# oma219/spumoni

Measured on AMD Instinct MI355X. Metric: reads/s PML classification, 200 bp reads vs 10-hap human index, higher is better.
Workload: dtype u64

## Files before the change

### spumoni_amd/csrc/spx_internal.h

```cpp
#pragma once
#include <hip/hip_runtime.h>

#include <memory>
#include <functional>
#include <mutex>
#include <string>
#include <vector>

#include "../../include/spumoni_gpu.h"
#include "spx_layout.h"

namespace spx {

void set_error(const char* fmt, ...);
int hip_fail(hipError_t e, const char* what, const char* file, int line);
int select_device(int device);

#define SPX_HIP(call)                                                        \
    do {                                                                     \
        hipError_t e_ = (call);                                              \
        if (e_ != hipSuccess) return spx::hip_fail(e_, #call, __FILE__, __LINE__); \
    } while (0)

struct QuietOnError {
// ... 59 lines not shown
    uint32_t* read_fail;
    const uint64_t* chunk_start;
    WalkState* reentry;
    uint64_t* vtop;
    uint32_t* pending;
    uint32_t round;
    uint32_t last_round;
};
constexpr uint32_t CHUNK_TOP = 0x80000000u, CHUNK_BOTTOM = 0x40000000u, CHUNK_ACTIVE = 0x20000000u;
constexpr uint32_t CHUNK_LEN_MASK = 0x1fffffffu;
constexpr int CHUNK_EXTRA_ROUNDS = 3;

struct BatchArgs {
    const uint8_t* seqs;
    const uint64_t* offs;
    uint64_t nreads;
    uint64_t total_chars;
    uint32_t* out_lengths;
    uint64_t* out_pointers;
    uint32_t* out_docs;
    spx_class* out_class;
    uint64_t bin_width;
    uint64_t bin_magic;
    uint64_t max_value_thr;
    WalkCounters* counters;
    uint32_t lanes_per_wave;
    uint32_t narrow;
    ChunkArgs ch;
    const uint32_t* only_flagged;
    const uint64_t* in_starts;
    uint64_t* len_mask;
    unsigned long long* claim;
    uint64_t len_mask_pairs;
};

}

struct spc_params;

namespace spx {
struct ArrayOwner {
    int device = 0;
    void* p[10] = {};
    ~ArrayOwner() {
        (void)hipSetDevice(device);
        for (void* a : p)
            if (a) (void)hipFree(a);
    }
};
}

struct spx_index {
    int device = 0;
    uint64_t n = 0, r = 0;
    bool has_samples = false, has_docs = false;
    spx::Row* rows = nullptr;
    uint32_t* q_alloc = nullptr;
    spx::JumpRow* dirrows = nullptr;
    char* fat = nullptr;
    uint32_t* fat_js = nullptr;
    spx::Aux* aux = nullptr;
    uint64_t* ss_by_run = nullptr;
    uint32_t* rundocs = nullptr;
    spx::LetterInfo* letters = nullptr;
    uint8_t* text = nullptr;
    uint64_t n_text = 0;
    static constexpr int NARR = 10;
    uint64_t arr_bytes[NARR] = {};
    std::shared_ptr<spx::ArrayOwner> owner;
    hipStream_t ctx_stream = nullptr;
    static constexpr int NDIGSCR = 15;
    hipEvent_t ev_dig = nullptr;
    hipStream_t dig_stream = nullptr;
    bool dig_used = false;
    spx::DevIndex view{};
    spx::WalkCounters* counters = nullptr;
    bool claim_used = false;
    hipEvent_t ev0 = nullptr, ev1 = nullptr, ev_done = nullptr;
    bool have_timing = false;
    hipStream_t last_stream = nullptr;
    uint64_t device_bytes = 0;
    int waves_per_cu = 0;
    int occ_blocks[8] = {};
    int num_cus = 0;
    int force_lanes_per_wave = 0;
    int force_digest_kernel = 0;
    int digest_parked = 0;
    uint8_t charhash[4] = {0, 0, 0, 0};
    char source_tag[128] = {0};
    static constexpr int PIPE_CHUNKS = 10;
    hipStream_t pipe_s[3] = {nullptr, nullptr, nullptr};
    hipEvent_t pipe_in[PIPE_CHUNKS] = {}, pipe_k[PIPE_CHUNKS] = {};
    std::mutex mu;
    std::mutex host_mu;
    struct Scratch {
        void* p = nullptr;
        size_t cap = 0;
        hipError_t grow(size_t bytes, void** out) {
            if (cap < bytes) {
                if (p) (void)hipFree(p);
                p = nullptr;
                cap = 0;
                const size_t want = bytes + bytes / 4 + 256;
                const hipError_t e = hipMalloc(&p, want);
                if (e != hipSuccess) return e;
                cap = want;
            }
            *out = p;
            return hipSuccess;
        }
        int reserve(size_t bytes, void** out) {
            SPX_HIP(grow(bytes, out));
            return SPX_OK;
        }
    };
    enum { S_SEQ, S_OFFS, S_LEN, S_PTR, S_DOC, S_CLASS, S_RAW, S_DIG_OFFS, S_GAP, S_SCAN,
           S_LINE_BYTES, S_LINE_START = S_LINE_BYTES + 3, S_TEXT = S_LINE_START + 3, S_COUNT = S_TEXT + 3 };
    static constexpr int reads_slot(int digest_kind) { return digest_kind ? S_RAW : S_SEQ; }
    Scratch scratch[S_COUNT];
    enum { C_DESC, C_ENDS, C_SEAMS, C_CKPT, C_FLAGS, C_FAIL, C_CNT, C_CUB, C_LEN_BITS, C_COUNT };
    Scratch chunk_scr[C_COUNT];
    Scratch digest_scr[NDIGSCR];
    enum { G_RAW, G_OFFS, G_DIG, G_DIG_OFFS, G_LEN, G_DOC, G_PTR, G_SET_STRIDE, G_COUNT = 2 * G_SET_STRIDE };
    Scratch stage_scr[G_COUNT];
    hipStream_t stage_s[2] = {nullptr, nullptr};
    struct Product {
        Scratch counters;
        hipEvent_t ev0 = nullptr, ev1 = nullptr;
        hipStream_t stream = nullptr;
        bool have = false, pending = false;
        uint64_t acc[6] = {};
        uint64_t error = 0;
        float ms = 0;
    };
    enum { V_MEDIUM, V_LONG, V_TILES, V_ACC, V_TABLE, V_OUT0, V_COUNT = V_OUT0 + 2 };
    Scratch vote_scr[V_COUNT];
    Product votes;
    enum { M_COUNTERS, M_BITS, M_PREFIX, M_CUB, M_MOFFS, M_OUT, M_OUT_DOCS, M_COUNT };
    Scratch mems_scr[M_COUNT];
    hipEvent_t ev_m[4] = {nullptr, nullptr, nullptr, nullptr};
    hipStream_t mems_stream = nullptr;
    bool have_mems = false, mems_pending = false, mems_ready = false, mems_ready_docs = false;
    uint64_t mems_capacity = 0, mems_ready_n = 0;
    uint64_t mems_acc[4] = {};
    float mems_ms = 0;
    Scratch place_scr[2];
    Product place;
    enum { H_OUT, H_COUNT };
    Scratch chain_scr[H_COUNT];
    Product chain;
    enum { L_CNT, L_GOFFS, L_GAPS, L_DESC, L_LIST, L_CUB, L_CHAINS, L_OUT, L_PRED, L_COUNT };
    Scratch align_scr[L_COUNT];
    Product align;
    hipEvent_t ev_align[3] = {nullptr, nullptr, nullptr};
    bool align_steps = false;
    float align_step_ms[4] = {};
    enum { TB_CNT, TB_GOFFS, TB_GAPS, TB_DESC, TB_LIST, TB_CUB, TB_PW, TB_POFFS, TB_PATH, TB_TRACE, TB_OCNT, TB_CHAINS, TB_OUT,
           TB_PRED, TB_OOFFS, TB_OPS, TB_EPW, TB_EPOFFS, TB_ERES, TB_ETRACE, TB_ENDS, TB_COUNT };
    Scratch cigar_scr[TB_COUNT];
    Product cigar;
    hipEvent_t ev_cigar[7] = {};
    bool cigar_phase[2] = {false, false};
    float cigar_step_ms[5] = {};
    uint64_t cigar_extra[4] = {};
    bool cigar_ready = false;
    uint64_t cigar_ready_n = 0, cigar_ready_reads = 0;
// ... 168 lines not shown
```

### spumoni_amd/csrc/spx_walk.hip

```cpp
#include <hipcub/hipcub.hpp>

#include <type_traits>

#include "spx_internal.h"

namespace spx {

namespace {

enum : uint32_t {
    P_READ = 0,
    P_CHARS = 1,
    P_LAND = 2,
    P_FAT = 3,
    P_QS = 4,
    P_DIR = 5,
    P_AUX = 6,
    P_SAMP = 7,
    P_FATJ = 8,
    P_DONE = 9,
    P_START = 10,
    P_CKPT = 11
};

// ... 870 lines not shown
    uint32_t k = (uint32_t)k_start;
    uint64_t off = 0;
    for (uint64_t guard = 0;; ++guard) {
        const Row row = row_at(ix, k);
        const uint32_t H = ix.compact ? crow_H(row) : row_H(row);
        if (t < n_text) text[t] = (uint8_t)H;
        uint32_t k0 = ix.compact ? crow_LFrun(row) : row_LFrun(row);
        uint64_t offp = (ix.compact ? (uint64_t)crow_LFoff(row) : row_LFoff(row)) + off;
        for (;;) {
            const Row r0 = row_at(ix, k0);
            const uint64_t len = ix.compact ? (uint64_t)crow_len(r0) : row_len(r0);
            if (offp < len || k0 >= ix.r) break;
            offp -= len;
            k0++;
        }
        if ((offp == 0 && !(ix.compact && crow_cont(row_at(ix, k0)))) || k0 >= ix.r) break;
        if (guard > ix.n) {
            atomicAdd(stuck, 1ull);
            break;
        }
        k = k0;
        off = offp;
        t -= 1;
    }
}

template <int MODE, bool DOC, bool COMPACT, bool NARROW, int CHUNK = 0>
int launch_lanes(spx_index* ix, const BatchArgs& args, hipStream_t stream, uint64_t items = 0, bool* wrote_lengths = nullptr) {
    if (CHUNK == 0) items = args.nreads;
    if (CHUNK == 0 && MODE == SPX_MODE_PML && args.out_lengths != nullptr && args.len_mask == nullptr) {
        set_error("internal: PML walk without prepare_len_mask");
        return SPX_E_ARG;
    }
    static const bool old_walk = getenv("SPX_OLD_WALK") != nullptr;
    const bool fast = COMPACT && args.only_flagged == nullptr && !old_walk && items < (1ull << 31);
    if (args.in_starts != nullptr && !(fast && CHUNK == 0)) {
        set_error("internal: parked reads (BatchArgs::in_starts) are taken by the plain k_walk_fast only");
        return SPX_E_ARG;
    }
    const int slot = (fast ? 4 : 0) + MODE * 2 + (DOC ? 1 : 0);
    if (ix->occ_blocks[slot] == 0) {
        int occ = 0;
        if (fast)
            SPX_HIP(hipOccupancyMaxActiveBlocksPerMultiprocessor(&occ, k_walk_fast<MODE, DOC, NARROW, 0>, WALK_TPB, 0));
        else
            SPX_HIP(hipOccupancyMaxActiveBlocksPerMultiprocessor(&occ, k_walk_lanes<MODE, DOC, COMPACT, NARROW, 0>, WALK_TPB, 0));
        ix->occ_blocks[slot] = occ < 1 ? 1 : occ;
    }
    if (ix->num_cus == 0) {
        hipDeviceProp_t prop;
        SPX_HIP(hipGetDeviceProperties(&prop, ix->device));
        ix->num_cus = prop.multiProcessorCount;
    }
    int occ = ix->occ_blocks[slot];
    constexpr bool SIDE = (MODE == SPX_MODE_MS) || DOC;
    const int auto_waves = ix->view.nletters > 16 ? (fast ? (SIDE ? 12 : 16) : 20) : (fast && SIDE ? 12 : 16);
    const int target_waves = ix->waves_per_cu > 0 ? ix->waves_per_cu : auto_waves;
    int want = target_waves / (WALK_TPB / 64);
    if (want < 1) want = 1;
    if (want < occ) occ = want;
    uint64_t grid = (uint64_t)occ * ix->num_cus;
    const uint64_t need = (items + WALK_TPB - 1) / WALK_TPB;
    BatchArgs a = args;
    a.lanes_per_wave = 64;
    bool small_batch = false;
    if (ix->force_lanes_per_wave > 0) {
        const uint64_t lpw = (uint64_t)(ix->force_lanes_per_wave > 64 ? 64 : ix->force_lanes_per_wave);
        a.lanes_per_wave = (uint32_t)lpw;
        const uint64_t waves_needed = (items + lpw - 1) / lpw;
        const uint64_t waves_resident = grid * (WALK_TPB / 64);
        const uint64_t waves = waves_needed < waves_resident ? waves_needed : waves_resident;
        grid = (waves + (WALK_TPB / 64) - 1) / (WALK_TPB / 64);
    } else if (need < grid) {
        small_batch = true;
        const uint64_t waves = (uint64_t)ix->num_cus * 4 * 2;
        uint64_t lpw = (items + waves - 1) / waves;
        if (lpw < 1) lpw = 1;
        if (lpw > 64) lpw = 64;
        a.lanes_per_wave = (uint32_t)lpw;
        grid = (items + lpw * 4 - 1) / (lpw * 4);
    }
    const bool dynamic = fast && CHUNK == 0 && ix->force_lanes_per_wave == 0 && !small_batch && items > grid * WALK_TPB;
    if (dynamic) {
        a.claim = &ix->counters->claim;
        if (ix->claim_used) SPX_HIP(hipMemsetAsync(a.claim, 0, sizeof(unsigned long long), stream));
        ix->claim_used = true;
    }
    if (!dynamic && ix->force_lanes_per_wave == 0 && need >= grid) {
        const uint64_t lanes_all = grid * WALK_TPB;
        const uint64_t rounds = (items + lanes_all - 1) / lanes_all;
        const uint64_t even = (items + rounds * WALK_TPB - 1) / (rounds * WALK_TPB);
        if (rounds <= 8 && even < grid && even * 8 >= grid * 7) grid = even;
    }
    if (grid == 0) grid = 1;
    if (fast) {
        if (dynamic)
            k_walk_fast<MODE, DOC, NARROW, 0, false, true><<<(unsigned)grid, WALK_TPB, 0, stream>>>(ix->view, a);
        else if (CHUNK == 2 || small_batch)
            k_walk_fast<MODE, DOC, NARROW, CHUNK, true><<<(unsigned)grid, WALK_TPB, 0, stream>>>(ix->view, a);
        else
            k_walk_fast<MODE, DOC, NARROW, CHUNK, false><<<(unsigned)grid, WALK_TPB, 0, stream>>>(ix->view, a);
        if (wrote_lengths) *wrote_lengths = MODE == SPX_MODE_PML;
    } else
        k_walk_lanes<MODE, DOC, COMPACT, NARROW, CHUNK><<<(unsigned)grid, WALK_TPB, 0, stream>>>(ix->view, a);
    SPX_HIP(hipGetLastError());
    return SPX_OK;
}


__global__ void k_chunk_count(const uint64_t* offs, uint64_t nreads, uint32_t L, int narrow, uint64_t* cnt,
                              uint32_t* read_fail, WalkCounters* counters) {
    const uint64_t q = blockIdx.x * (uint64_t)WALK_TPB + threadIdx.x;
    if (q > nreads) return;
    if (q == nreads) {
        cnt[q] = 0;
        return;
    }
    const uint64_t base = offs[q], m = offs[q + 1] - base;
    cnt[q] = m ? (base + m - 1) / L - base / L + 1 : 0;
    read_fail[q] = 0;
    if (narrow && m >= 65536) atomicAdd(&counters->error, 1ull);
}

__global__ void k_chunk_fill(const uint64_t* offs, uint64_t nreads, uint32_t L, const uint64_t* chunk_start,
                             ChunkDesc* desc, uint64_t* nchunks) {
    const uint64_t q = blockIdx.x * (uint64_t)WALK_TPB + threadIdx.x;
    if (q >= nreads) return;
    if (q == 0) *nchunks = chunk_start[nreads];
    const uint64_t base = offs[q], end = offs[q + 1];
    uint64_t c = chunk_start[q];
    for (uint64_t a = base; a < end; ++c) {
        uint64_t e = (a / L + 1) * L;
        if (e > end) e = end;
        ChunkDesc d;
        d.gend = e;
        d.len = (uint32_t)(e - a) | (e == end ? CHUNK_TOP : 0u) | (a == base ? CHUNK_BOTTOM : 0u);
        d.rd = (uint32_t)q;
        desc[c] = d;
        a = e;
    }
}

__global__ void k_chunk_scan(ChunkArgs ch, uint64_t nreads, uint32_t round, uint32_t last, WalkCounters* counters) {
    const uint64_t q = blockIdx.x * (uint64_t)WALK_TPB + threadIdx.x;
    if (q >= nreads) return;
    const uint64_t cs = ch.chunk_start[q], ce = ch.chunk_start[q + 1];
    if (ce - cs < 2) return;
    ChunkDesc* desc = const_cast<ChunkDesc*>(ch.desc);
    uint64_t j = round == 1 ? ce - 1 : ch.vtop[q];
    if (j == cs) return;
    if (round > 1) desc[j - 1].len &= ~CHUNK_ACTIVE;
    while (j > cs) {
        const uint64_t nx = j - 1;
        const SeamRec sr = ch.seams[nx];
        j = nx;
        if (nx == cs || (sr.met & 1)) continue;
        if (!last) {
            WalkState st = sr.ext;
            const ChunkDesc below = desc[nx - 1];
            const SeamRec old = ch.seams[nx - 1];
            st.flags = (uint32_t)(old.t - (below.gend - (below.len & CHUNK_LEN_MASK)));
            ch.reentry[nx - 1] = st;
            desc[nx - 1].len = below.len | CHUNK_ACTIVE;
            atomicAdd(&ch.pending[round + 1], 1u);
        }
        break;
// ... 545 lines not shown
```

### spumoni_amd/csrc/spx_walk_fast.inc

```

enum : uint32_t { Q_LAND = 0, Q_FAT = 1, Q_STEP = 2, Q_READ = 3, Q_CHARS = 4, Q_FATJ = 5, Q_QS = 6, Q_DIR = 7, Q_DONE = 8, Q_SAMP = 9, Q_START = 10, Q_WANT = 11 };
enum : uint32_t {
    F_EMB = 1,
    F_NOROW = 2,
    F_QUIRK = 4,
    F_WIDE = 16,
    F_FADD = 32,
    F_HAVEC = 64,
    F_SAMPD = 128
};
enum : uint32_t { A_STEP = 1, A_EMIT = 2, A_DECIDE = 4 };
#ifndef SPX_STEP_REPS
#define SPX_STEP_REPS 2
#endif
constexpr int STEP_REPS = SPX_STEP_REPS;
constexpr uint32_t OFF_LAST32 = 0xffffffffu;
#ifndef SPX_CHUNK_CLAIM
#define SPX_CHUNK_CLAIM 64
#endif
constexpr uint32_t CHUNK_CLAIM = SPX_CHUNK_CLAIM;
static_assert(CHUNK_CLAIM >= 64, "a claim covers at least one iteration's worst case: 64 lanes ending a read each");

__device__ __forceinline__ uint32_t dpp_swap1(uint32_t v) { return (uint32_t)__builtin_amdgcn_mov_dpp((int)v, 0xB1, 0xf, 0xf, true); }

struct alignas(16) HotLetter {
    uint32_t bmul;
    uint32_t present;
    uint64_t fat0;
};

__device__ __forceinline__ void lf_target_ct(uint32_t LFrun, uint32_t LFoff, uint32_t cums, uint32_t off, uint32_t& k0,
                                             uint32_t& offp, uint32_t& t_out) {
    lf_target_c(LFrun, LFoff, cums, off, k0, offp);
    const uint32_t t = k0 - LFrun;
    t_out = (t < 4 && off <= 126) ? t : 4u;
}

template <int MODE, bool DOC, bool NARROW, int CHUNK = 0, bool EARLY = false, bool DYN = false>
__global__ void __launch_bounds__(WALK_TPB) k_walk_fast(const DevIndex ix, const BatchArgs b) {
    constexpr bool AUX = (MODE == SPX_MODE_MS) || DOC;
    constexpr bool PML = MODE == SPX_MODE_PML;
    if (CHUNK == 2 && b.ch.round > 1 && b.ch.pending[b.ch.round] == 0) return;
    __shared__ HotLetter s_hot[256];
#ifndef SPX_PGRP
#define SPX_PGRP 16
#endif
    constexpr int PGRP = SPX_PGRP, PROW = WALK_TPB + 1;
    constexpr int PLPG = PGRP / 2, PNG = 64 / PLPG;
    __shared__ uint64_t s_ptrs[MODE == SPX_MODE_MS && CHUNK != 2 ? PGRP * PROW : 1];
    constexpr bool DSTAGE = PML && DOC && CHUNK != 2;
    constexpr int DGRP = 32, DROW = DGRP + 2;
    __shared__ uint16_t s_docs[DSTAGE ? WALK_TPB * DROW : 1];
    const LetterInfo* const s_let = ix.letters;
    __shared__ uint32_t s_win[8 * WALK_TPB];
    const char* const rows_b = reinterpret_cast<const char*>(ix.rows);
    const char* const fat_b = reinterpret_cast<const char*>(ix.fat);
    const uint32_t fs = ix.fat_stride;
    const bool lrow = !AUX && fs == 32 && ix.aux == nullptr;
    for (int t = threadIdx.x; t < 256; t += blockDim.x) {
        const LetterInfo li = ix.letters[t];
        s_hot[t] = HotLetter{li.bmul, li.qbeg != li.qend ? 1u : 0u, (uint64_t)(uintptr_t)(fat_b + li.fbase * fs)};
    }
    __syncthreads();
    const char* const dir_b = reinterpret_cast<const char*>(ix.dirrows);
    const char* const fatj_b = reinterpret_cast<const char*>(ix.fat_js);
    const char* const q_b = reinterpret_cast<const char*>(ix.Q);
    const char* const seq_b = reinterpret_cast<const char*>(b.seqs);
    const char* const off_b = reinterpret_cast<const char*>(b.offs);
    const uint32_t R = ix.r;
    const uint32_t fs_shift = fs == 32 ? 5 : 4;
    const bool want_class = PML && CHUNK == 0 && b.out_class != nullptr;
    const bool want_len = PML && CHUNK != 2 && b.out_lengths != nullptr;
    const uint32_t lpw = b.lanes_per_wave;
    const uint32_t nlanes = (uint32_t)((((uint64_t)gridDim.x * blockDim.x) >> 6) * lpw);
    const uint32_t nitems = CHUNK ? (uint32_t)*b.ch.nchunks : (uint32_t)b.nreads;
    const uint64_t ch_org = CHUNK ? b.offs[0] : 0;
    uint8_t* const ch_flags = CHUNK ? b.ch.flags - (ch_org & ~7ull) : nullptr;
    WalkState* const ch_ckpt = CHUNK ? b.ch.ckpt - (ch_org >> CKPT_SHIFT) : nullptr;
    const char* const item_b = CHUNK ? reinterpret_cast<const char*>(b.ch.desc) : off_b;
    constexpr uint32_t ITEM_BYTES = CHUNK ? sizeof(ChunkDesc) : 8;
    const uint32_t tid = threadIdx.x;
    static_assert(!DYN || (CHUNK == 0 && !EARLY), "only the plain, full launch deals its reads on demand");
    uint32_t w_n0 = 0, w_e0 = 0, w_n1 = 0, w_e1 = 0;
    bool w_pend = false;
    bool w_dry = false;
    uint32_t w_wait = DYN ? (uint32_t)((((uint64_t)blockIdx.x * blockDim.x + tid) >> 6) & 31u) + 1u : 0u;
    unsigned long long claimed = 0;

    uint32_t rd = (uint32_t)((((uint64_t)blockIdx.x * blockDim.x + tid) >> 6) * lpw) + (tid & 63);
    uint32_t ph = (rd < nitems && (tid & 63) < lpw) ? Q_READ : Q_DONE;
    const char* addr = ph == Q_READ ? item_b + (uint64_t)rd * ITEM_BYTES : item_b;
    uint32_t seen = 0;
    uint64_t fb = 0;
    uint32_t fl = 0;
    uint32_t c = 0;
    uint64_t base = 0, ibase = 0;
    uint32_t m = 0, x = 0;
    int32_t wi = -1;
    uint64_t q0 = 0, q1 = 0;
    uint32_t k = 0, off = 0;
    uint32_t length = 0;
    uint64_t mbits = 0;
    uint32_t nr = 0;
    uint32_t bin_lo = 0, bin_max = 0, above = 0, below = 0;
    uint64_t sum_max = 0;
    uint64_t sample = 0;
    uint32_t doc = 0;
    uint32_t w_jumps = 0, w_pred = 0, w_rows = 0, w_dir = 0, w_again = 0;
    uint32_t tlimit = 0xffffffffu;
    V16 cka{0, 0, 0, 0}, ckb{0, 0, 0, 0};

#define WIN_AT(w) ((s_win[((uint32_t)(w) >> 2) * WALK_TPB + tid] >> (((uint32_t)(w) & 3) * 8)) & 0xffu)
#define CUR_C c
#define COUNT(var, cond) (var += (uint32_t)__popcll(__builtin_amdgcn_ballot_w64(cond)))

    V16 ga{0, 0, 0, 0}, gb{0, 0, 0, 0};
    uint32_t side_doc = 0;
    Aux side_aux{0, 0};
    uint64_t side_in = 0;
    auto issue_gather = [&]() {
        ga = V16{0, 0, 0, 0};
        gb = V16{0, 0, 0, 0};
#ifndef SPX_PAIR_MIN
#define SPX_PAIR_MIN 24
#endif
        constexpr int pair_min = EARLY ? 65 : SPX_PAIR_MIN;
        if ((int)__popcll(__builtin_amdgcn_ballot_w64(ph != Q_DONE && (fl & F_WIDE))) < pair_min) {
            if (ph != Q_DONE) {
                ga = *reinterpret_cast<const V16*>(addr);
                if (fl & F_WIDE) gb = *reinterpret_cast<const V16*>(addr + 16);
            }
        } else
        {
            typedef uint32_t u32x4 __attribute__((ext_vector_type(4), aligned(4)));
            typedef const __attribute__((address_space(1))) u32x4* GV16;
            const bool odd = tid & 1;
            const bool live = ph != Q_DONE;
            const uint32_t w_own = (live && (fl & F_WIDE)) ? 16u : 0u;
            const uint64_t au = (uint64_t)(uintptr_t)(live ? addr : rows_b);
            const uint64_t pu = u64of(dpp_swap1((uint32_t)au), dpp_swap1((uint32_t)(au >> 32))) + 16;
            const uint32_t w_for = dpp_swap1(w_own);
            const uint64_t a1 = odd ? pu : au, a2 = odd ? au : pu;
            const bool do1 = odd ? w_for != 0 : live, do2 = odd ? live : w_for != 0;
            uint32_t r1x = 0, r1y = 0, r1z = 0, r1w = 0, r2x = 0, r2y = 0, r2z = 0, r2w = 0;
            if (do1) {
                const u32x4 t = *(GV16)(uintptr_t)a1;
                r1x = t.x, r1y = t.y, r1z = t.z, r1w = t.w;
            }
            if (do2) {
                const u32x4 t = *(GV16)(uintptr_t)a2;
                r2x = t.x, r2y = t.y, r2z = t.z, r2w = t.w;
            }
            ga = V16{odd ? r2x : r1x, odd ? r2y : r1y, odd ? r2z : r1z, odd ? r2w : r1w};
            const uint32_t zx = dpp_swap1(odd ? r1x : r2x), zy = dpp_swap1(odd ? r1y : r2y), zz = dpp_swap1(odd ? r1z : r2z),
                           zw = dpp_swap1(odd ? r1w : r2w);
            gb = V16{w_own ? zx : 0u, w_own ? zy : 0u, w_own ? zz : 0u, w_own ? zw : 0u};
        }
        side_doc = 0;
        side_aux = Aux{0, 0};
        side_in = 0;
        claimed = 0;
        if (CHUNK == 0 && b.in_starts != nullptr && ph == Q_READ) side_in = b.in_starts[rd];
        if (DOC && ph == Q_SAMP) side_doc = ix.rundocs[k];
        if (AUX && ph == Q_DIR) side_aux = ix.aux[length];
        if (DYN && w_pend && (tid & 63) == 0) claimed = atomicAdd(b.claim, (unsigned long long)CHUNK_CLAIM);
    };
    if (EARLY) issue_gather();
    while (__builtin_amdgcn_ballot_w64(ph != Q_DONE) != 0) {
        if (!EARLY) issue_gather();
        uint32_t act = 0, hd = 0;
        uint32_t rflag = 0;
        bool pred_ev = false;
        uint32_t d_trun = 0, d_toff = 0, d_srun = 0, d_soff = 0, d_bits = 0;
        Aux d_aux{0, 0};
        bool d_lrow = false;
        uint64_t fbits = 0;
        uint32_t fxi = 0;
        bool flush = false;
        bool pflush = false, pheld = false, pheld_end = false;
        uint32_t pfxi = 0;
        uint64_t phold = 0;
        COUNT(w_rows, ph == Q_LAND);
        COUNT(w_dir, ph == Q_FAT || (ph >= Q_FATJ && ph <= Q_DIR));

        if (ph == Q_LAND) {
            const uint32_t len = ga.x & 0xffffu;
            const uint32_t o = off == OFF_LAST32 ? len - 1 : off;
            if (o >= len) {
                off = o - len;
                k++;
                addr += sizeof(Row32);
            } else {
                off = o;
                q0 = u64of(ga.x, ga.y);
                q1 = u64of(ga.z, ga.w);
                fl = (fl & ~F_NOROW) | F_EMB;
                act = A_STEP;
            }
        } else if (ph == Q_FAT) {
            const uint32_t hq = ga.x;
            const uint32_t w1l = ga.z, w1h = ga.w;
            const bool nosucc = (w1h >> 29) & 1, esc = (w1h >> 30) & 1;
            const bool quirk = fl & F_QUIRK;
            const bool found = nosucc || hq > k || (quirk && hq == k);
            if (found && !esc && !quirk) {
                d_trun = hq - (w1l & 0x7ffffu);
                d_toff = ((w1l >> 20) | (w1h << 12)) & 0xffffu;
                d_srun = ga.y;
                const uint32_t sfield = (w1h >> 4) & 0xffffu;
                const bool ps = (w1h >> 28) & 1;
                d_soff = ps ? sfield : 0u;
                d_bits = ((w1h >> 20) & 0xffu) | ((uint32_t)ps << 8) | ((uint32_t)nosucc << 9) | ((w1h >> 31) << 10) |
                         ((ps ? 0u : (sfield & 0xffu)) << 16);
                if (AUX) d_aux = Aux{u64of(gb.x, gb.y), u64of(gb.z, gb.w)};
                d_lrow = lrow;
                act = A_DECIDE;
            } else if (!found && (w1l & (uint32_t)FAT_SINGLE) && !(fl & F_FADD)) {
                fl |= F_FADD;
                addr += fs;
            } else if (found && esc && !quirk) {
                length = ga.y;
                fl |= F_WIDE;
                ph = Q_DIR;
                addr = dir_b + (uint64_t)length * sizeof(JumpRow);
            } else {
                const uint64_t grp = ((uint64_t)(addr - fat_b) >> fs_shift) >> FJ_SHIFT;
                length = (uint32_t)grp & 3;
                fl &= ~F_WIDE;
                ph = Q_FATJ;
                addr = fatj_b + ((grp * 4) & ~15ull);
            }
        } else if (ph == Q_STEP) {
            act = A_STEP;
        } else if (ph != Q_DONE && ph != Q_SAMP && (!DYN || ph != Q_WANT)) {
            if (ph == Q_READ) {
                if (CHUNK) {
                    m = ga.z & CHUNK_LEN_MASK;
                    base = u64of(ga.x, ga.y) - m;
                    seen = 0;
                    fb = 0;
                    if (CHUNK == 2 && (((ga.z >> 29) & 4) || (b.ch.round > 1 && !((ga.z >> 29) & 1)))) m = 0;
                } else {
                    base = u64of(ga.x, ga.y);
                    m = (uint32_t)(u64of(ga.z, ga.w) - base);
                }
                ibase = (CHUNK == 0 && b.in_starts != nullptr) ? side_in : base;
                if (m == 0) {
                    if (want_class) b.out_class[rd] = spx_class{0, 0, 0};
                    rd += DYN ? 0u : nlanes;
                    ph = DYN ? Q_WANT : (rd < nitems ? Q_READ : Q_DONE);
                    addr = DYN ? rows_b : item_b + (uint64_t)rd * ITEM_BYTES;
                } else {
                    if (NARROW && CHUNK == 0 && m >= 65536) atomicAdd(&b.counters->error, 1ull);
                    x = m;
                    length = 0;
                    sample = ix.init_sample;
                    doc = ix.init_doc;
                    k = ix.init_k;
                    off = (uint32_t)ix.init_off;
                    q0 = ix.init_row.q0;
                    q1 = ix.init_row.q1;
                    fl = 0;
                    wi = -1;
                    mbits = 0;
                    nr = m;
                    if (want_class) {
                        const uint32_t w = (uint32_t)b.bin_width;
                        const uint32_t q = w > 1 ? (uint32_t)__umul64hi((uint64_t)m, b.bin_magic) : m;
                        const uint32_t nb = q > 0 ? q : 1;
                        bin_lo = (nb - 1) * w;
                        bin_max = above = below = 0;
                        sum_max = 0;
                    }
                    act = A_STEP;
                    if (CHUNK == 2) {
                        ph = Q_START;
                        addr = reinterpret_cast<const char*>(b.ch.round > 1 ? b.ch.reentry + rd : b.ch.ends + rd + 1);
                        fl = F_WIDE;
                        act = 0;
                    }
                }
            } else if (ph == Q_CHARS) {
                s_win[0 * WALK_TPB + tid] = ga.x;
                s_win[1 * WALK_TPB + tid] = ga.y;
                s_win[2 * WALK_TPB + tid] = ga.z;
                s_win[3 * WALK_TPB + tid] = ga.w;
                s_win[4 * WALK_TPB + tid] = gb.x;
                s_win[5 * WALK_TPB + tid] = gb.y;
                s_win[6 * WALK_TPB + tid] = gb.z;
                s_win[7 * WALK_TPB + tid] = gb.w;
                ph = Q_STEP;
                act = A_STEP;
            } else if (CHUNK == 2 && ph == Q_START) {
                k = ga.x;
                length = ga.y;
                {
                    const uint64_t offp = u64of(ga.z, ga.w);
                    off = offp == OFF_END ? OFF_LAST32 : (uint32_t)offp;
                }
                sample = u64of(gb.x, gb.y);
                doc = gb.z;
                tlimit = b.ch.round > 1 ? gb.w : 0xffffffffu;
                ph = Q_LAND;
                addr = rows_b + (uint64_t)k * sizeof(Row32);
                fl = F_WIDE;
                {
                    const char* const cp = reinterpret_cast<const char*>(ch_ckpt + ((base + m - 1) >> CKPT_SHIFT));
                    cka = *reinterpret_cast<const V16*>(cp);
                    ckb = *reinterpret_cast<const V16*>(cp + 16);
                }
            } else if (ph == Q_FATJ) {
                const uint32_t lo = (length & 2) ? ga.z : ga.x, hi = (length & 2) ? ga.w : ga.y;
                length = (length & 1) ? hi : lo;
                fl |= F_WIDE;
                ph = Q_QS;
                addr = q_b + (uint64_t)length * 4;
            } else if (ph == Q_QS) {
                const uint32_t e[8] = {ga.x, ga.y, ga.z, ga.w, gb.x, gb.y, gb.z, gb.w};
                const uint32_t room_q = s_let[CUR_C].qend - length;
                uint32_t skip = 0;
#pragma unroll
                for (int t = 0; t < 8; ++t) skip += ((uint32_t)t < room_q && e[t] < k) ? 1u : 0u;
                length += skip;
                if (skip < 8) {
                    ph = Q_DIR;
                    addr = dir_b + (uint64_t)length * sizeof(JumpRow);
                } else {
// ... 62 lines not shown
            if (dec) {
                if (below_thr && ((d_bits >> 10) & 1)) atomicAdd(&b.counters->error, 1ull);
                const bool last = below_thr && !psame;
                k = d_srun - (last ? 1u : 0u);
                off = last ? OFF_LAST32 : d_soff - (below_thr ? 1u : 0u);
                hd = last ? ((d_bits >> 16) & 0xffu) : (d_bits & 0xffu);
                if (MODE == SPX_MODE_MS) sample = below_thr ? aux_se(d_aux) : aux_ss(d_aux);
                if (DOC) doc = below_thr ? (aux_docs(d_aux) >> 16) : (aux_docs(d_aux) & 0xffffu);
                length = 0;
                fl = (fl & ~(F_EMB | F_QUIRK)) | ((d_lrow && !last) ? F_EMB : 0u);
                rflag = 3;
                act = A_EMIT;
            }
        }

#pragma unroll
        for (int rep = 0; rep < STEP_REPS; ++rep) {
            if (rep > 0 && __builtin_amdgcn_ballot_w64(act != 0) == 0) break;
            bool jumped = false;
            if (act & A_STEP) {
                const bool havec = fl & F_HAVEC;
                if (!havec && wi < 0) {
                    const uint64_t g = ibase + x - 1;
                    const uint64_t end4 = (g + 4) & ~3ull;
                    const uint64_t wbase = end4 >= 32 ? end4 - 32 : 0;
                    wi = (int32_t)(g - wbase);
                    ph = Q_CHARS;
                    addr = seq_b + wbase;
                    fl = (fl | F_WIDE) & ~F_EMB;
                    act = 0;
                } else {
                    const uint32_t cw = WIN_AT(wi < 0 ? 0 : wi);
                    c = havec ? c : cw;
                    wi -= havec ? 0 : 1;
                    const HotLetter hl = s_hot[c];
                    const uint32_t H = (uint32_t)q1 & 0xffu;
                    const bool eq = k < R && H == c;
                    const bool lf = eq && (c < 128 || ((q1 >> 8) & 1));
                    const bool present = hl.present != 0;
                    const bool go_land = eq && (fl & F_NOROW);
                    const bool go_fat = !go_land && present && !lf;
                    const bool go_samp = AUX && !go_land && lf && c >= 128 && !(fl & F_SAMPD);
                    const bool fin = !(go_land || go_fat || go_samp);
                    const bool lfin = fin && present;
                    uint32_t tk, toff, t;
                    lf_target_ct((uint32_t)(q0 >> 32), (uint32_t)(q0 >> 16) & 0xffffu, (uint32_t)(q1 >> 32), off, tk, toff, t);
                    t = lfin ? t : 4u;
                    const char* a_land = rows_b + (uint64_t)k * sizeof(Row32);
                    const char* a_fat = reinterpret_cast<const char*>((uintptr_t)hl.fat0) + (uint64_t)fat_block(k, hl.bmul) * fs;
                    addr = go_land ? a_land : (go_fat ? a_fat : addr);
                    ph = go_land ? Q_LAND : (go_fat ? Q_FAT : ph);
                    if (go_samp) {
                        addr = reinterpret_cast<const char*>(MODE == SPX_MODE_MS ? (const void*)(ix.ss_by_run + k) : (const void*)(ix.rundocs + k));
                        ph = Q_SAMP;
                    }
                    k = lfin ? tk : k;
                    off = lfin ? toff : off;
                    if (fin && !present) {
                        k = s_let[c].frun;
                        off = (uint32_t)s_let[c].foff;
                        if (MODE == SPX_MODE_MS) {
                            sample = 0;
                            if (DOC) doc = ix.doc_at0;
                        }
                    }
                    if (MODE == SPX_MODE_MS) sample -= (lfin && c < 128) ? 1u : 0u;
                    length = (lfin && c < 128) ? length + 1 : (fin ? 0u : length);
                    if (CHUNK) rflag = (lfin && c < 128) ? 0u : (lfin ? 3u : (MODE == SPX_MODE_MS ? 3u : 1u));
                    jumped = go_fat || (lfin && c >= 128);
                    hd = t < 2 ? ((uint32_t)(q1 >> (16 + 8 * t)) & 0xffu) : 0u;
                    uint32_t nf = fl & ~(F_HAVEC | F_SAMPD | (t == 0 ? 0u : F_EMB));
                    nf = go_fat ? ((nf & ~(F_QUIRK | F_FADD | F_WIDE)) | (eq ? F_QUIRK : 0u) | ((AUX || lrow) ? F_WIDE : 0u)) : nf;
                    nf = go_land ? (nf | F_WIDE | F_HAVEC) : nf;
                    nf = go_samp ? ((nf | F_HAVEC) & ~F_WIDE) : nf;
                    fl = nf;
                    act = fin ? A_EMIT : 0u;
                }
            }
            COUNT(w_jumps, jumped);
            if (CHUNK == 2) COUNT(w_again, (act & A_EMIT) != 0);
            if (act & A_EMIT) {
                const uint32_t xi = x - 1;
                x = xi;
                bool met = false;
                if (CHUNK == 2) {
                    const uint64_t gi = base + xi;
                    seen |= rflag;
                    ch_flags[gi] = (uint8_t)rflag;
                    if (PML) {
                        if (NARROW)
                            reinterpret_cast<uint16_t*>(b.out_lengths)[gi] = (uint16_t)length;
                        else
                            b.out_lengths[gi] = length;
                    } else {
                        b.out_pointers[gi] = sample;
                    }
                    if (DOC) {
                        if (NARROW)
                            reinterpret_cast<uint16_t*>(b.out_docs)[gi] = (uint16_t)doc;
                        else
                            b.out_docs[gi] = doc;
                    }
                    const uint64_t my_off = off == OFF_LAST32 ? OFF_END : (uint64_t)off;
                    if (xi != 0 && (gi & ((1u << CKPT_SHIFT) - 1)) == 0) {
                        if (cka.x == k && u64of(cka.z, cka.w) == my_off && xi <= tlimit) {
                            SeamRec sr;
                            sr.t = gi;
                            sr.met = 1 | (b.ch.round << 8);
                            sr.reset_above = seen;
                            sr.ext = WalkState{k, length, my_off, sample, doc, seen};
                            sr.spec_length = cka.y;
                            sr.spec_doc = ckb.z;
                            sr.spec_sample = u64of(ckb.x, ckb.y);
                            b.ch.seams[rd] = sr;
                            met = true;
                        } else {
                            const char* const cp = reinterpret_cast<const char*>(ch_ckpt + ((gi >> CKPT_SHIFT) - 1));
                            cka = *reinterpret_cast<const V16*>(cp);
                            ckb = *reinterpret_cast<const V16*>(cp + 16);
                        }
                    } else if (xi == 0) {
                        SeamRec sr;
                        sr.t = base;
                        sr.met = b.ch.round << 8;
                        sr.reset_above = seen;
                        sr.ext = WalkState{k, length, my_off, sample, doc, seen};
                        sr.spec_length = 0;
                        sr.spec_doc = 0;
                        sr.spec_sample = 0;
                        b.ch.seams[rd] = sr;
                    }
                }
                if (CHUNK == 1) {
                    const uint64_t gi = base + xi;
                    seen |= rflag;
                    const uint32_t slot = (uint32_t)gi & 7;
                    fb |= (uint64_t)rflag << (slot * 8);
                    if (slot == 0 || xi == 0) {
                        const uint64_t g8 = gi & ~7ull;
                        if (g8 >= base && g8 + 7 < base + m) {
                            *reinterpret_cast<uint64_t*>(ch_flags + g8) = fb;
                        } else {
#pragma unroll
                            for (int t8 = 0; t8 < 8; ++t8)
                                if (g8 + t8 >= gi && g8 + t8 < base + m) ch_flags[g8 + t8] = (uint8_t)(fb >> (t8 * 8));
                        }
                        fb = 0;
                    }
                    if (xi == 0 || ((base + xi) & ((1u << CKPT_SHIFT) - 1)) == 0) {
                        const WalkState ws{k, length, off == OFF_LAST32 ? OFF_END : (uint64_t)off, sample, doc, seen};
                        if (xi == 0)
                            b.ch.ends[rd] = ws;
                        else
                            ch_ckpt[(base + xi) >> CKPT_SHIFT] = ws;
                    }
                }
                if (MODE == SPX_MODE_MS && CHUNK != 2) {
                    const uint32_t slot = ((uint32_t)base + xi) & (PGRP - 1);
                    const uint64_t pv = (sample & 0xffffffffffffull) | (DOC ? (uint64_t)doc << 48 : 0ull);
                    if (pflush) {
                        phold = pv;
                        pheld = true;
                        pheld_end = xi == 0;
                    } else {
                        s_ptrs[slot * PROW + tid] = pv;
                        if (slot == 0 || xi == 0) {
                            pflush = true;
                            pfxi = xi;
                        }
                    }
                }
                if (DSTAGE) {
                    const uint32_t slot = ((uint32_t)base + xi) & (DGRP - 1);
                    if (pflush) {
                        phold = doc;
                        pheld = true;
                        pheld_end = xi == 0;
                    } else {
                        s_docs[tid * DROW + slot] = (uint16_t)doc;
                        if (slot == 0 || xi == 0) {
                            pflush = true;
                            pfxi = xi;
                        }
                    }
                }
                if (PML && CHUNK != 2) {
                    mbits = (mbits << 1) | (length == 0 ? 1u : 0u);
                    if ((xi & 63) == 0) {
                        fbits = mbits;
                        fxi = xi;
                        flush = true;
                        mbits = 0;
                    }
                }
                if (want_class) {
                    if (xi < bin_lo) {
                        const bool ab = bin_max >= b.max_value_thr;
                        above += ab ? 1u : 0u;
                        below += ab ? 0u : 1u;
                        sum_max += bin_max;
                        bin_max = 0;
                        bin_lo -= (uint32_t)b.bin_width;
                    }
                    bin_max = length > bin_max ? length : bin_max;
                }
                if (xi == 0 || (CHUNK == 2 && met)) {
                    if (want_class) {
                        const bool ab = bin_max >= b.max_value_thr;
                        b.out_class[rd] = spx_class{sum_max + bin_max, above + (ab ? 1u : 0u), below + (ab ? 0u : 1u)};
                    }
                    rd += DYN ? 0u : nlanes;
                    ph = DYN ? Q_WANT : (rd < nitems ? Q_READ : Q_DONE);
                    addr = DYN ? rows_b : item_b + (uint64_t)rd * ITEM_BYTES;
                    fl = 0;
                    act = 0;
                } else {
                    const bool stand = fl & F_EMB;
                    const bool head_only = !stand && hd != 0 && rep + 1 < STEP_REPS;
                    const bool ld = !stand && !head_only;
                    q0 = stand ? u64of(gb.x, gb.y) : q0;
                    q1 = stand ? u64of(gb.z, gb.w) : (head_only ? (uint64_t)hd : q1);
                    fl = (fl & ~(F_EMB | F_NOROW)) | (head_only ? F_NOROW : 0u) | (ld ? F_WIDE : 0u);
                    const char* a_land = rows_b + (uint64_t)k * sizeof(Row32);
                    addr = ld ? a_land : addr;
                    ph = ld ? Q_LAND : ph;
                    act = ld ? 0u : A_STEP;
                }
            }
        }
        if (act != 0) {
            ph = Q_STEP;
            addr = rows_b;
            fl &= ~(F_WIDE | F_EMB);
        }
        if (DYN) {
            if (w_pend) {
                const uint64_t c0 = (uint64_t)nlanes + u64of((uint32_t)__builtin_amdgcn_readfirstlane((int)(uint32_t)claimed),
                                                             (uint32_t)__builtin_amdgcn_readfirstlane((int)(uint32_t)(claimed >> 32)));
                const uint64_t c1 = c0 + CHUNK_CLAIM;
                w_n1 = (uint32_t)(c0 < nitems ? c0 : nitems);
                w_e1 = (uint32_t)(c1 < nitems ? c1 : nitems);
                w_dry = c1 >= nitems;
                w_pend = false;
            }
            if (w_n0 == w_e0) {
                w_n0 = w_n1;
                w_e0 = w_e1;
                w_n1 = w_e1 = 0;
            }
            const uint64_t wants = __builtin_amdgcn_ballot_w64(ph == Q_WANT);
            if (wants != 0) {
                const uint32_t j = __builtin_amdgcn_mbcnt_hi((uint32_t)(wants >> 32), __builtin_amdgcn_mbcnt_lo((uint32_t)wants, 0u));
                const uint32_t have0 = w_e0 - w_n0, have1 = w_e1 - w_n1, nw = (uint32_t)__popcll(wants);
                const bool over = !w_pend && w_dry;
                if (ph == Q_WANT) {
                    const bool got = j < have0 + have1;
                    rd = j < have0 ? w_n0 + j : w_n1 + (j - have0);
                    ph = got ? Q_READ : (over ? Q_DONE : Q_WANT);
                    addr = got ? item_b + (uint64_t)rd * ITEM_BYTES : rows_b;
                }
                const uint32_t t0 = nw < have0 ? nw : have0, t1 = (nw - t0) < have1 ? (nw - t0) : have1;
                w_n0 += t0;
                w_n1 += t1;
                if (nw > have0 + have1) w_wait = 0;
                if (w_n0 == w_e0) {
                    w_n0 = w_n1;
                    w_e0 = w_e1;
                    w_n1 = w_e1 = 0;
                }
            }
            w_wait -= w_wait != 0 ? 1u : 0u;
            w_pend = !w_dry && w_wait == 0 && w_n1 == w_e1 && (w_e0 - w_n0) < 64u;
        }
        if (EARLY) issue_gather();
        if (MODE == SPX_MODE_MS && CHUNK != 2) {
            const uint32_t lane = tid & 63;
            uint64_t todo = __builtin_amdgcn_ballot_w64(pflush);
            while (todo != 0) {
                while (todo != 0) {
                    uint32_t src = 64;
#pragma unroll
                    for (int kx = 0; kx < PNG; ++kx) {
                        if (todo != 0) {
                            const uint32_t l = (uint32_t)__builtin_ctzll(todo);
                            todo &= todo - 1;
                            src = (lane / PLPG) == (uint32_t)kx ? l : src;
                        }
                    }
                    const bool valid = src < 64;
                    const uint32_t from = valid ? src : lane;
                    const uint32_t sxi = (uint32_t)__shfl((int)pfxi, (int)from);
                    const uint32_t sm = (uint32_t)__shfl((int)m, (int)from);
                    const uint64_t sbase = u64of((uint32_t)__shfl((int)(uint32_t)base, (int)from), (uint32_t)__shfl((int)(uint32_t)(base >> 32), (int)from));
                    const uint32_t e2 = (lane % PLPG) * 2;
                    const uint64_t lo = sbase + sxi, hi = sbase + sm;
                    const uint64_t p0 = (lo & ~(uint64_t)(PGRP - 1)) + e2;
                    const uint64_t v0 = s_ptrs[e2 * PROW + (tid & ~63u) + from];
                    const uint64_t v1 = s_ptrs[(e2 + 1) * PROW + (tid & ~63u) + from];
                    const bool ok0 = valid && p0 >= lo && p0 < hi, ok1 = valid && p0 + 1 >= lo && p0 + 1 < hi;
                    const uint64_t q0p = (uint64_t)((int64_t)(v0 << 16) >> 16), q1p = (uint64_t)((int64_t)(v1 << 16) >> 16);
                    if (ok0 && ok1) {
                        __builtin_nontemporal_store(q0p, b.out_pointers + p0);
                        __builtin_nontemporal_store(q1p, b.out_pointers + p0 + 1);
                    } else if (ok0) {
                        b.out_pointers[p0] = q0p;
                    } else if (ok1) {
                        b.out_pointers[p0 + 1] = q1p;
                    }
                    if (DOC) {
                        const uint32_t d0 = (uint32_t)(v0 >> 48), d1 = (uint32_t)(v1 >> 48);
                        if (NARROW) {
                            uint16_t* const dp = reinterpret_cast<uint16_t*>(b.out_docs) + p0;
                            if (ok0 && ok1)
                                *reinterpret_cast<H16x2*>(dp) = H16x2{d0 | (d1 << 16)};
                            else if (ok0)
                                dp[0] = (uint16_t)d0;
                            else if (ok1)
                                dp[1] = (uint16_t)d1;
                        } else {
                            if (ok0 && ok1)
                                *reinterpret_cast<U32x2*>(b.out_docs + p0) = U32x2{d0, d1};
                            else if (ok0)
                                b.out_docs[p0] = d0;
                            else if (ok1)
                                b.out_docs[p0 + 1] = d1;
                        }
                    }
                }
                pflush = false;
                if (pheld) {
                    s_ptrs[(PGRP - 1) * PROW + tid] = phold;
                    pheld = false;
                    pflush = pheld_end;
                    pfxi = 0;
                }
                todo = __builtin_amdgcn_ballot_w64(pflush);
            }
        }
        if (DSTAGE) {
            const uint32_t lane = tid & 63;
            uint64_t todo = __builtin_amdgcn_ballot_w64(pflush);
            while (todo != 0) {
                while (todo != 0) {
                    uint32_t src = 64;
#pragma unroll
                    for (int kx = 0; kx < 8; ++kx) {
                        if (todo != 0) {
                            const uint32_t l = (uint32_t)__builtin_ctzll(todo);
                            todo &= todo - 1;
                            src = (lane >> 3) == (uint32_t)kx ? l : src;
                        }
// ... 8 lines not shown
                    const uint64_t p0 = (lo & ~(uint64_t)(DGRP - 1)) + e4;
                    const uint16_t* const sp = &s_docs[((tid & ~63u) + from) * DROW + e4];
                    const uint32_t w0 = *reinterpret_cast<const uint32_t*>(sp), w1 = *reinterpret_cast<const uint32_t*>(sp + 2);
                    if (valid && p0 >= lo && p0 + 4 <= hi) {
                        if (NARROW)
                            *reinterpret_cast<H16x4*>(reinterpret_cast<uint16_t*>(b.out_docs) + p0) = H16x4{u64of(w0, w1)};
                        else
                            *reinterpret_cast<U32x4*>(b.out_docs + p0) = U32x4{w0 & 0xffffu, w0 >> 16, w1 & 0xffffu, w1 >> 16};
                    } else if (valid) {
#pragma unroll
                        for (int t4 = 0; t4 < 4; ++t4) {
                            const uint32_t dv = ((t4 & 2 ? w1 : w0) >> ((t4 & 1) * 16)) & 0xffffu;
                            if (p0 + t4 >= lo && p0 + t4 < hi) {
                                if (NARROW)
                                    reinterpret_cast<uint16_t*>(b.out_docs)[p0 + t4] = (uint16_t)dv;
                                else
                                    b.out_docs[p0 + t4] = dv;
                            }
                        }
                    }
                }
                pflush = false;
                if (pheld) {
                    s_docs[tid * DROW + (DGRP - 1)] = (uint16_t)phold;
                    pheld = false;
                    pflush = pheld_end;
                    pfxi = 0;
                }
                todo = __builtin_amdgcn_ballot_w64(pflush);
            }
        }
        if (PML && want_len) {
            uint64_t todo = __builtin_amdgcn_ballot_w64(flush);
            const uint32_t lane = tid & 63;
            while (todo != 0) {
                const uint32_t l = (uint32_t)__builtin_ctzll(todo);
                todo &= todo - 1;
                const uint64_t wbits = u64of((uint32_t)__builtin_amdgcn_readlane((int)(uint32_t)fbits, l),
                                             (uint32_t)__builtin_amdgcn_readlane((int)(uint32_t)(fbits >> 32), l));
                const uint32_t wxi = (uint32_t)__builtin_amdgcn_readlane((int)fxi, l);
                const uint32_t wnr = (uint32_t)__builtin_amdgcn_readlane((int)nr, l);
                const uint32_t wm = (uint32_t)__builtin_amdgcn_readlane((int)m, l);
                const uint64_t wbase = u64of((uint32_t)__builtin_amdgcn_readlane((int)(uint32_t)base, l),
                                             (uint32_t)__builtin_amdgcn_readlane((int)(uint32_t)(base >> 32), l));
                const uint32_t cnt = wm - wxi;
                const uint64_t t = wbits >> lane;
                const uint32_t v = t != 0 ? (uint32_t)__builtin_ctzll(t) : wnr - (wxi + lane);
                if (lane < cnt) {
                    if (NARROW)
                        reinterpret_cast<uint16_t*>(b.out_lengths)[wbase + wxi + lane] = (uint16_t)v;
                    else
                        b.out_lengths[wbase + wxi + lane] = v;
                }
            }
        }
        if (PML && CHUNK != 2 && flush) nr = fbits != 0 ? fxi + (uint32_t)__builtin_ctzll(fbits) : nr;
    }
#undef WIN_AT
#undef CUR_C
#undef COUNT
    if ((tid & 63) == 0) {
        if (CHUNK == 2) {
            atomicAdd(&b.counters->reserved0, (unsigned long long)w_again);
        } else {
            atomicAdd(&b.counters->jumps, (unsigned long long)w_jumps);
            atomicAdd(&b.counters->pred_jumps, (unsigned long long)w_pred);
        }
        atomicAdd(&b.counters->row_loads, (unsigned long long)w_rows);
        atomicAdd(&b.counters->dir_loads, (unsigned long long)w_dir);
    }
    (void)sample;
    (void)doc;
    (void)s_ptrs;
    (void)s_docs;
    (void)seen;
    (void)fb;
    (void)ch_flags;
    (void)ch_ckpt;
    (void)tlimit;
    (void)cka;
    (void)ckb;
    (void)w_again;
    (void)w_n0, (void)w_e0, (void)w_n1, (void)w_e1, (void)w_pend, (void)w_dry, (void)w_wait, (void)claimed;
    if (CHUNK != 2 && blockIdx.x == 0 && tid == 0) atomicAdd(&b.counters->steps, (unsigned long long)(b.offs[b.nreads] - b.offs[0]));
}
```

Measured before the change: 1.085 billion.

## Stage per-read PML outputs in LDS and flush claimed chunks coalesced

In the dynamic-claim PML kernel without documents, per-read class results and the match bit-words are held in shared-memory slots tied to each claimed chunk. Once every read of a chunk has finished, the wave writes the classes and expands the length bits into out_lengths in a coalesced pass over aligned 64-element lines, instead of each lane issuing scattered stores. Launch code now queries the occupancy of the dynamic kernel, which carries extra shared memory, and shrinks the grid to match. The change adds substantial LDS use, which may lower occupancy, plus bookkeeping and atomics in shared memory.

Result: faster. 1.179 billion, median of 6 (+8.7%).

```diff
diff --git a/spumoni_amd/csrc/spx_internal.h b/spumoni_amd/csrc/spx_internal.h
--- a/spumoni_amd/csrc/spx_internal.h
+++ b/spumoni_amd/csrc/spx_internal.h
@@ -165,6 +165,7 @@
     uint64_t device_bytes = 0;
     int waves_per_cu = 0;
     int occ_blocks[8] = {};
+    int occ_blocks_dyn[4] = {};
     int num_cus = 0;
     int force_lanes_per_wave = 0;
     int force_digest_kernel = 0;
diff --git a/spumoni_amd/csrc/spx_walk.hip b/spumoni_amd/csrc/spx_walk.hip
--- a/spumoni_amd/csrc/spx_walk.hip
+++ b/spumoni_amd/csrc/spx_walk.hip
@@ -976,6 +976,16 @@
     }
     const bool dynamic = fast && CHUNK == 0 && ix->force_lanes_per_wave == 0 && !small_batch && items > grid * WALK_TPB;
     if (dynamic) {
+        const int dslot = MODE * 2 + (DOC ? 1 : 0);
+        if (ix->occ_blocks_dyn[dslot] == 0) {
+            int occ_d = 0;
+            SPX_HIP(hipOccupancyMaxActiveBlocksPerMultiprocessor(&occ_d, k_walk_fast<MODE, DOC, NARROW, 0, false, true>, WALK_TPB, 0));
+            ix->occ_blocks_dyn[dslot] = occ_d < 1 ? 1 : occ_d;
+        }
+        if (ix->occ_blocks_dyn[dslot] < occ) {
+            occ = ix->occ_blocks_dyn[dslot];
+            grid = (uint64_t)occ * ix->num_cus;
+        }
         a.claim = &ix->counters->claim;
         if (ix->claim_used) SPX_HIP(hipMemsetAsync(a.claim, 0, sizeof(unsigned long long), stream));
         ix->claim_used = true;
diff --git a/spumoni_amd/csrc/spx_walk_fast.inc b/spumoni_amd/csrc/spx_walk_fast.inc
--- a/spumoni_amd/csrc/spx_walk_fast.inc
+++ b/spumoni_amd/csrc/spx_walk_fast.inc
@@ -40,6 +40,7 @@
 __global__ void __launch_bounds__(WALK_TPB) k_walk_fast(const DevIndex ix, const BatchArgs b) {
     constexpr bool AUX = (MODE == SPX_MODE_MS) || DOC;
     constexpr bool PML = MODE == SPX_MODE_PML;
+    constexpr bool STAGE = DYN && PML && !DOC;
     if (CHUNK == 2 && b.ch.round > 1 && b.ch.pending[b.ch.round] == 0) return;
     __shared__ HotLetter s_hot[256];
 #ifndef SPX_PGRP
@@ -53,6 +54,12 @@
     __shared__ uint16_t s_docs[DSTAGE ? WALK_TPB * DROW : 1];
     const LetterInfo* const s_let = ix.letters;
     __shared__ uint32_t s_win[8 * WALK_TPB];
+    constexpr int CSLOTS = 3, CWAVE = CSLOTS * 64, CALL = (WALK_TPB / 64) * CWAVE;
+    constexpr uint32_t C_NONE = 0xffffffffu;
+    __shared__ uint64_t s_cbase[STAGE ? CALL : 1];
+    __shared__ uint64_t s_cword[STAGE ? CALL : 1];
+    __shared__ uint64_t s_ccls[STAGE ? 2 * CALL : 1];
+    __shared__ uint8_t s_clen[STAGE ? CALL : 1];
     const char* const rows_b = reinterpret_cast<const char*>(ix.rows);
     const char* const fat_b = reinterpret_cast<const char*>(ix.fat);
     const uint32_t fs = ix.fat_stride;
@@ -90,6 +97,33 @@
     uint32_t rd = (uint32_t)((((uint64_t)blockIdx.x * blockDim.x + tid) >> 6) * lpw) + (tid & 63);
     uint32_t ph = (rd < nitems && (tid & 63) < lpw) ? Q_READ : Q_DONE;
     const char* addr = ph == Q_READ ? item_b + (uint64_t)rd * ITEM_BYTES : item_b;
+    const uint32_t cw0 = (tid >> 6) * CWAVE;
+    uint32_t cidx = C_NONE;
+    uint32_t c_first[CSLOTS] = {0, 0, 0}, c_n[CSLOTS] = {0, 0, 0}, c_left[CSLOTS] = {0, 0, 0};
+    uint32_t w_cb0 = 0, w_cb1 = 0;
+    bool w_cv0 = false, w_cv1 = false, w_ct0 = false, w_ct1 = false;
+    auto take_slot = [&](uint32_t first, uint32_t count, uint32_t& cb, bool& cv) {
+        const uint32_t fs_ = c_n[0] == 0 ? 0u : (c_n[1] == 0 ? 1u : (c_n[2] == 0 ? 2u : 3u));
+        cv = fs_ < (uint32_t)CSLOTS;
+        if (cv) {
+#pragma unroll
+            for (int s = 0; s < CSLOTS; ++s) {
+                c_first[s] = fs_ == (uint32_t)s ? first : c_first[s];
+                c_n[s] = fs_ == (uint32_t)s ? count : c_n[s];
+                c_left[s] = fs_ == (uint32_t)s ? count : c_left[s];
+            }
+            cb = fs_ * 64 - first;
+            s_clen[cw0 + fs_ * 64 + (threadIdx.x & 63)] = 0;
+        }
+    };
+    static_assert(CSLOTS == 3, "the slots' scalars are written out by hand");
+    if (STAGE) {
+        const uint32_t f0 = (uint32_t)__builtin_amdgcn_readfirstlane((int)(rd - (tid & 63)));
+        c_first[0] = f0;
+        c_n[0] = c_left[0] = f0 < nitems ? (nitems - f0 < 64u ? nitems - f0 : 64u) : 0u;
+        cidx = ph == Q_READ ? (tid & 63) : C_NONE;
+        s_clen[cw0 + (tid & 63)] = 0;
+    }
     uint32_t seen = 0;
     uint64_t fb = 0;
     uint32_t fl = 0;
@@ -243,6 +277,7 @@
                 } else {
                     base = u64of(ga.x, ga.y);
                     m = (uint32_t)(u64of(ga.z, ga.w) - base);
+                    if (STAGE && cidx != C_NONE) s_cbase[cw0 + cidx] = base;
                 }
                 ibase = (CHUNK == 0 && b.in_starts != nullptr) ? side_in : base;
                 if (m == 0) {
@@ -471,6 +506,8 @@
             if (act & A_EMIT) {
                 const uint32_t xi = x - 1;
                 x = xi;
+                const bool staged = STAGE && cidx != C_NONE && m <= 64;
+                (void)staged;
                 bool met = false;
                 if (CHUNK == 2) {
                     const uint64_t gi = base + xi;
@@ -576,9 +613,14 @@
                 if (PML && CHUNK != 2) {
                     mbits = (mbits << 1) | (length == 0 ? 1u : 0u);
                     if ((xi & 63) == 0) {
-                        fbits = mbits;
-                        fxi = xi;
-                        flush = true;
+                        if (STAGE && staged) {
+                            s_cword[cw0 + cidx] = mbits;
+                            s_clen[cw0 + cidx] = (uint8_t)m;
+                        } else {
+                            fbits = mbits;
+                            fxi = xi;
+                            flush = true;
+                        }
                         mbits = 0;
                     }
                 }
@@ -596,7 +638,12 @@
                 if (xi == 0 || (CHUNK == 2 && met)) {
                     if (want_class) {
                         const bool ab = bin_max >= b.max_value_thr;
-                        b.out_class[rd] = spx_class{sum_max + bin_max, above + (ab ? 1u : 0u), below + (ab ? 0u : 1u)};
+                        if (STAGE && staged) {
+                            s_ccls[2 * (cw0 + cidx)] = sum_max + bin_max;
+                            s_ccls[2 * (cw0 + cidx) + 1] = u64of(above + (ab ? 1u : 0u), below + (ab ? 0u : 1u));
+                        } else {
+                            b.out_class[rd] = spx_class{sum_max + bin_max, above + (ab ? 1u : 0u), below + (ab ? 0u : 1u)};
+                        }
                     }
                     rd += DYN ? 0u : nlanes;
                     ph = DYN ? Q_WANT : (rd < nitems ? Q_READ : Q_DONE);
@@ -622,6 +669,101 @@
             addr = rows_b;
             fl &= ~(F_WIDE | F_EMB);
         }
+        if (STAGE) {
+            const bool ended = ph == Q_WANT && cidx != C_NONE;
+            if (__builtin_amdgcn_ballot_w64(ended) != 0) {
+                uint32_t ready = 0;
+#pragma unroll
+                for (int s = 0; s < CSLOTS; ++s) {
+                    c_left[s] -= (uint32_t)__popcll(__builtin_amdgcn_ballot_w64(ended && (cidx >> 6) == (uint32_t)s));
+                    ready |= (c_n[s] != 0 && c_left[s] == 0) ? 1u << s : 0u;
+                }
+                cidx = ended ? C_NONE : cidx;
+                while (ready != 0) {
+                    const uint32_t s = (uint32_t)__builtin_ctz(ready);
+                    ready &= ready - 1;
+                    const uint32_t cn = s == 0 ? c_n[0] : (s == 1 ? c_n[1] : c_n[2]);
+                    const uint32_t cf = s == 0 ? c_first[0] : (s == 1 ? c_first[1] : c_first[2]);
+                    c_n[0] = s == 0 ? 0u : c_n[0];
+                    c_n[1] = s == 1 ? 0u : c_n[1];
+                    c_n[2] = s == 2 ? 0u : c_n[2];
+                    const uint32_t lane = tid & 63, so = cw0 + s * 64;
+                    if (want_class && lane < cn && s_clen[so + lane] != 0) {
+                        const uint64_t cv = s_ccls[2 * (so + lane) + 1];
+                        b.out_class[cf + lane] = spx_class{s_ccls[2 * (so + lane)], (uint32_t)cv, (uint32_t)(cv >> 32)};
+                    }
+                    if (want_len) {
+                        const int64_t lo = (int64_t)s_cbase[so];
+                        const int64_t hi = (int64_t)s_cbase[so + cn - 1] + s_clen[so + cn - 1];
+                        const int64_t skew = (int64_t)(((uintptr_t)b.out_lengths >> (NARROW ? 1 : 2)) & 63);
+                        const int64_t e00 = ((lo + skew) & ~63ll) - skew;
+                        uint32_t ci = 0;
+                        int64_t cb = lo;
+                        if (hi - e00 <= 64 * 64) {
+                            const bool mine = lane < cn;
+                            const int64_t bi = mine ? (int64_t)s_cbase[so + lane] : hi;
+                            const int64_t bn = lane + 1 < cn ? (int64_t)s_cbase[so + lane + 1] : hi;
+                            const uint32_t li = s_clen[so + lane];
+                            const uint64_t wi = s_cword[so + lane];
+                            const bool holds = mine && bn > bi;
+                            const uint64_t hmask = __builtin_amdgcn_ballot_w64(holds);
+                            const uint32_t rank = __builtin_amdgcn_mbcnt_hi((uint32_t)(hmask >> 32), __builtin_amdgcn_mbcnt_lo((uint32_t)hmask, 0u));
+                            unsigned long long* const bits = reinterpret_cast<unsigned long long*>(&s_ccls[2 * so]);
+                            bits[lane] = 0;
+                            if (holds) {
+                                const uint32_t q = (uint32_t)(bi - e00);
+                                atomicOr(&bits[q >> 6], 1ull << (q & 63));
+                                s_cbase[so + rank] = (uint64_t)bi;
+                                s_clen[so + rank] = (uint8_t)li;
+                                s_cword[so + rank] = wi;
+                            }
+                            const uint64_t mown = atomicOr(&bits[lane], 0ull);
+                            const uint32_t nlines = (uint32_t)((hi - e00 + 63) >> 6);
+                            uint32_t before = 0;
+                            for (uint32_t ln = 0; ln < nlines; ++ln) {
+                                const uint64_t mk = u64of((uint32_t)__builtin_amdgcn_readlane((int)(uint32_t)mown, (int)ln),
+                                                          (uint32_t)__builtin_amdgcn_readlane((int)(uint32_t)(mown >> 32), (int)ln));
+                                const uint32_t upto = before + __builtin_amdgcn_mbcnt_hi((uint32_t)(mk >> 32), __builtin_amdgcn_mbcnt_lo((uint32_t)mk, 0u)) +
+                                                      (uint32_t)((mk >> lane) & 1);
+                                before += (uint32_t)__popcll(mk);
+                                const int64_t e = e00 + (int64_t)ln * 64 + lane;
+                                if (upto != 0) {
+                                    const uint64_t p = (uint64_t)(e - (int64_t)s_cbase[so + upto - 1]);
+                                    const uint32_t cm = s_clen[so + upto - 1];
+                                    if (p < cm) {
+                                        const uint64_t t = s_cword[so + upto - 1] >> p;
+                                        const uint32_t v = t != 0 ? (uint32_t)__builtin_ctzll(t) : cm - (uint32_t)p;
+                                        if (NARROW)
+                                            reinterpret_cast<uint16_t*>(b.out_lengths)[e] = (uint16_t)v;
+                                        else
+                                            b.out_lengths[e] = v;
+                                    }
+                                }
+                            }
+                        } else
+                        for (int64_t e0 = e00; e0 < hi; e0 += 64) {
+                            const int64_t e = e0 + lane;
+                            while (ci + 1 < cn) {
+                                const int64_t nb = (int64_t)s_cbase[so + ci + 1];
+                                if (nb > e) break;
+                                cb = nb;
+                                ++ci;
+                            }
+                            const uint64_t p = (uint64_t)(e - cb);
+                            const uint32_t cm = s_clen[so + ci];
+                            if (p < cm) {
+                                const uint64_t t = s_cword[so + ci] >> p;
+                                const uint32_t v = t != 0 ? (uint32_t)__builtin_ctzll(t) : cm - (uint32_t)p;
+                                if (NARROW)
+                                    reinterpret_cast<uint16_t*>(b.out_lengths)[e] = (uint16_t)v;
+                                else
+                                    b.out_lengths[e] = v;
+                            }
+                        }
+                    }
+                }
+            }
+        }
         if (DYN) {
             if (w_pend) {
                 const uint64_t c0 = (uint64_t)nlanes + u64of((uint32_t)__builtin_amdgcn_readfirstlane((int)(uint32_t)claimed),
@@ -631,22 +773,37 @@
                 w_e1 = (uint32_t)(c1 < nitems ? c1 : nitems);
                 w_dry = c1 >= nitems;
                 w_pend = false;
+                w_cv1 = w_ct1 = false;
             }
             if (w_n0 == w_e0) {
                 w_n0 = w_n1;
                 w_e0 = w_e1;
                 w_n1 = w_e1 = 0;
+                w_cb0 = w_cb1;
+                w_cv0 = w_cv1;
+                w_ct0 = w_ct1;
             }
             const uint64_t wants = __builtin_amdgcn_ballot_w64(ph == Q_WANT);
             if (wants != 0) {
                 const uint32_t j = __builtin_amdgcn_mbcnt_hi((uint32_t)(wants >> 32), __builtin_amdgcn_mbcnt_lo((uint32_t)wants, 0u));
                 const uint32_t have0 = w_e0 - w_n0, have1 = w_e1 - w_n1, nw = (uint32_t)__popcll(wants);
                 const bool over = !w_pend && w_dry;
+                if (STAGE) {
+                    if (have0 != 0 && !w_ct0) {
+                        take_slot(w_n0, have0, w_cb0, w_cv0);
+                        w_ct0 = true;
+                    }
+                    if (nw > have0 && have1 != 0 && !w_ct1) {
+                        take_slot(w_n1, have1, w_cb1, w_cv1);
+                        w_ct1 = true;
+                    }
+                }
                 if (ph == Q_WANT) {
                     const bool got = j < have0 + have1;
                     rd = j < have0 ? w_n0 + j : w_n1 + (j - have0);
                     ph = got ? Q_READ : (over ? Q_DONE : Q_WANT);
                     addr = got ? item_b + (uint64_t)rd * ITEM_BYTES : rows_b;
+                    if (STAGE) cidx = (got && (j < have0 ? w_cv0 : w_cv1)) ? rd + (j < have0 ? w_cb0 : w_cb1) : C_NONE;
                 }
                 const uint32_t t0 = nw < have0 ? nw : have0, t1 = (nw - t0) < have1 ? (nw - t0) : have1;
                 w_n0 += t0;
@@ -656,6 +813,9 @@
                     w_n0 = w_n1;
                     w_e0 = w_e1;
                     w_n1 = w_e1 = 0;
+                    w_cb0 = w_cb1;
+                    w_cv0 = w_cv1;
+                    w_ct0 = w_ct1;
                 }
             }
             w_wait -= w_wait != 0 ? 1u : 0u;
@@ -830,5 +990,7 @@
     (void)ckb;
     (void)w_again;
     (void)w_n0, (void)w_e0, (void)w_n1, (void)w_e1, (void)w_pend, (void)w_dry, (void)w_wait, (void)claimed;
+    (void)cidx, (void)c_first, (void)c_n, (void)c_left, (void)w_cb0, (void)w_cb1, (void)w_cv0, (void)w_cv1, (void)w_ct0, (void)w_ct1;
+    (void)take_slot, (void)cw0, (void)s_cbase, (void)s_cword, (void)s_ccls, (void)s_clen;
     if (CHUNK != 2 && blockIdx.x == 0 && tid == 0) atomicAdd(&b.counters->steps, (unsigned long long)(b.offs[b.nreads] - b.offs[0]));
 }
```
